# tangxyw/RecAlgorithm

Hardware: AMD Instinct MI355X
Metric: CTR examples/sec (train step fwd+bwd+TF1-Adam), batch 4096/GPU, 26 fields x emb16 (higher is better)
Workload: dtype f32; 1 GPU; DCN 3-layer CrossNet + MLP 512,256,128; 26 fields x emb16; batch 4096/GPU; data_batches=32, global_batch=4096, fields=26, emb_dim=16, embedding_rows=2790871, launch=hipGraph replay, parallelism=single

## Files before the change

recalgorithm_amd/_lib.py:

```python
from __future__ import annotations

import ctypes
import os
import re

from . import _abi
from ._abi import RecalgoError

_HERE = os.path.dirname(os.path.abspath(__file__))
LIB_PATH = os.environ.get("RECALGO_HIP_LIB") or os.path.join(_HERE, "librecalgo_hip.so")

P = ctypes.c_void_p


def _versioned(header: str):
    abi = _abi.read(header)
    defines = [c for c in abi.constants if re.fullmatch(r"RECALGO_(?:[A-Z0-9]+_)?ABI_VERSION", c)]
    queries = [f for f in abi.functions if re.fullmatch(r"recalgo_(?:[a-z0-9]+_)?abi_version", f)]
    if len(defines) != 1 or queries != [defines[0].lower()]:
        raise RecalgoError(f"include/{header}: a header of HEADERS has exactly one RECALGO_[<KEY>_]ABI_VERSION define and the "
                           f"one function recalgo_[<key>_]abi_version of the same key; found {defines} and {queries}")
    abi.version, abi.version_query = abi.constants[defines[0]], queries[0]
    abi.label = defines[0][len("RECALGO_"):-len("_VERSION")].replace("_", " ")
    return abi


HEADERS = {h: _versioned(h) for h in ("recalgo.h", "recalgo_cgc.h", "recalgo_wide.h", "recalgo_bst.h",
                                              "recalgo_res.h")}
MORE_HEADERS = {"recalgo_dien.h": _versioned("recalgo_dien.h")}
SERVING_HEADERS = {h: _versioned(h) for h in ("recalgo_serve.h", "recalgo_metrics.h", "recalgo_sumstep.h",
                                                      "recalgo_ragged.h", "recalgo_afm.h")}
ABI = HEADERS["recalgo.h"]
SIGNATURES = ABI.functions
STRUCTS = ABI.structs
CONSTANTS = ABI.constants
ABI_VERSION = ABI.version
_lib = None


def all_headers() -> dict:
    return {**HEADERS, **MORE_HEADERS}


def every_header() -> dict:
    return {**all_headers(), **SERVING_HEADERS}


def launch_errcheck(name: str):
    def errcheck(rc, func=None, args=None):
        check(rc, name)
        return rc
    return errcheck


# ... 30 lines not shown
```

recalgorithm_amd/csrc/sparse.hip:

```cpp
#include <cstddef>
#include <cstdlib>

#include "deferred.h"

#ifndef RECALGO_APPLY_WGS
#define RECALGO_APPLY_WGS 4
#endif
#ifndef RECALGO_APPLY_LDS_KEYS
#define RECALGO_APPLY_LDS_KEYS 2048
#endif
#ifndef RECALGO_APPLY_KU
#define RECALGO_APPLY_KU 8
#endif

namespace {

constexpr int kThreads = 256;
constexpr int kMaxSources = RECALGO_SCATTER_MAX_SOURCES;
using recalgo_deferred::kLrRing;
constexpr unsigned kLdsKeys = RECALGO_APPLY_LDS_KEYS;
constexpr unsigned kMaxSeg = kThreads;
constexpr unsigned kSlots = 512;
constexpr unsigned kLongSeg = 48;
constexpr unsigned kMaxLong = 64;
constexpr unsigned kCatchReq = 128;
constexpr unsigned long long kPadKey = ~0ull;
// ... 191 lines not shown

constexpr int kPrepSources = 4;
struct PrepareArgs {
    SrcDev S;
    SrcDev Sx[kPrepSources - 1];
    unsigned n_src;
    unsigned nreq_x[kPrepSources - 1];
    unsigned catch_end[kPrepSources];
    unsigned count_end[kPrepSources];
    unsigned* total;
    unsigned nb_log2, cs;
    Deferred D;
    Deferred D1;
    const long long* step;
    int step_off;
    unsigned K;
    unsigned n_req;
    unsigned b_catch, b_comp, b_count, b_sweep;
    long long rows, rows1;
    int period;
    unsigned passes, passes1;
    unsigned bshift, bshift1;
    int sweeping;
};

__device__ __forceinline__ long long request_row_linear(const SrcDev& S, unsigned r) {
    const unsigned e = r / S.F, f = r - e * S.F;
    return request_row(S, e, f);
}

__device__ __forceinline__ bool claim_row(int* last_step, long long row, int target, int* s_out) {
    const int s = __hip_atomic_load(&last_step[row], __ATOMIC_RELAXED, __HIP_MEMORY_SCOPE_AGENT);
    if (s > 0 && s < target && atomicCAS(&last_step[row], s, -s) == s) {
        *s_out = s;
        return true;
    }
    return false;
}

struct Claims {
    int* row; int* s;
    int* row2; int* s2;
    int* won;
    unsigned* hist;
    unsigned* n;
};
// ... 168 lines not shown
    int s = 0, old = 0;
    bool lag = false;
    long long row = -1;
    if (active && r < n_req) {
        row = request_row_linear(S, r);
        if (row >= 0 && row < n_rows && !(A.sweeping && (int)((row >> (8 + bshift)) % A.period) == cidx)) {
            s = __hip_atomic_load(&D.last_step[row], __ATOMIC_RELAXED, __HIP_MEMORY_SCOPE_AGENT);
            lag = s > 0 && s < target;
        }
    }
    if (lag) old = atomicCAS(&D.last_step[row], s, -s);
    unsigned slot = 0;
    if (lag) {
        slot = atomicAdd(C.n, 1u);
        C.row[slot] = (int)row;
        C.s[slot] = s;
    }
    __syncthreads();
    replay_claims(D, K, target, C, recalgo_deferred::lr_window(D.lr_ring, target), lag, slot, old, s);
}

__global__ __launch_bounds__(kThreads, 8) void sparse_prepare_kernel(PrepareArgs A) {
    extern __shared__ __attribute__((aligned(16))) unsigned lds_u[];
    const int target = A.D.last_step ? (int)(A.step[0] + A.step_off) : 0;
    const int cidx = A.period > 0 ? target % A.period : 0;
    if (blockIdx.x < A.b_catch) {
        if (A.n_src > 1) {
            unsigned si = 0, b0 = 0;
#pragma unroll
            for (int i = 1; i < kPrepSources; ++i)
                if ((unsigned)i < A.n_src && blockIdx.x >= A.catch_end[i - 1]) { si = i; b0 = A.catch_end[i - 1]; }
            SrcDev S = A.S;
            unsigned n_req = A.n_req;
#pragma unroll
            for (int i = 1; i < kPrepSources; ++i)
                if (si == (unsigned)i) { S = A.Sx[i - 1]; n_req = A.nreq_x[i - 1]; }
            catchup_requests(A, S, n_req, A.D, A.K, (blockIdx.x - b0) * kCatchReq + threadIdx.x, threadIdx.x < kCatchReq, A.rows, A.bshift,
                             cidx, target, claims_carve(lds_u));
            return;
        }
        catchup_requests(A, A.S, A.n_req, A.D, A.K, blockIdx.x * kCatchReq + threadIdx.x, threadIdx.x < kCatchReq, A.rows, A.bshift, cidx,
                         target, claims_carve(lds_u));
        return;
    }
    if (blockIdx.x < A.b_comp) {
        catchup_requests(A, A.S, A.n_req, A.D1, 1, (blockIdx.x - A.b_catch) * kThreads + threadIdx.x, true, A.rows1, A.bshift1, cidx,
// ... 14 lines not shown
            for (int i = 1; i < kPrepSources; ++i)
                if (si == (unsigned)i) S = A.Sx[i - 1];
            cb -= b0;
        }
        const unsigned li = cb * kThreads + threadIdx.x;
        unsigned e, f;
        const long long row = li < S.n ? slot_row(S, li, &e, &f) : -1;
        unsigned slot;
        const EqInfo eq = tile_equal(row >= 0 ? (unsigned)row : 0xffffffffu, hkey, mask, &slot);
        if (row >= 0 && eq.before == 0) atomicAdd(&A.total[(size_t)bucket_of((unsigned)row, A.nb_log2) << A.cs], 1u);
        return;
    }
    if (target <= 0) return;
    const Claims C = claims_carve(lds_u);
    if (blockIdx.x < A.b_sweep) {
        const recalgo_deferred::LrWindow W = recalgo_deferred::lr_window(A.D.lr_ring, target);
        const long long wg = blockIdx.x - A.b_count, nwg = A.b_sweep - A.b_count;
        sweep_units(A.D, A.K, A.passes, [&](unsigned pu) { return sweep_unit_row(cidx, A.period, A.bshift, wg + (long long)pu * nwg); },
                    A.rows, target, C, W);
        return;
    }
    {
        const recalgo_deferred::LrWindow W = recalgo_deferred::lr_window(A.D1.lr_ring, target);
        const long long wg = blockIdx.x - A.b_sweep, nwg = (long long)gridDim.x - A.b_sweep;
        sweep_units(A.D1, 1, A.passes1, [&](unsigned pu) { return sweep_unit_row(cidx, A.period, A.bshift1, wg + (long long)pu * nwg); },
                    A.rows1, target, C, W);
    }
}

struct PlaceArgs {
    SrcDev src[kMaxSources];
    int n_src;
    unsigned n_total;
    const unsigned* total; unsigned* cursor;
    unsigned cs;
    uint4* sched;
    const unsigned* offs_g; int prescanned;
    float* hdr;
    float* lr_ring; float* lr_ring1;
    const long long* step; int step_off;
    float lr, b1, b2;
    unsigned long long* keys;
    float* partials;
    float* partials1;
    unsigned nb_log2;
    unsigned KV, L;
    int stage_ok;
// ... 688 lines not shown

RECALGO_EXPORT int64_t recalgo_scatter_plan_header_bytes(int nb_log2) {
    if (!nb_ok(nb_log2)) return 0;
    return (32 + 2 * ((1ll << nb_log2) << counter_shift())) * (int64_t)sizeof(unsigned);
}

RECALGO_EXPORT int recalgo_scatter_plan_scan(void* plan_workspace, int64_t plan_requests, int nb_log2, recalgo_plan_scan_t* out) {
    RECALGO_REQUIRE(plan_workspace != nullptr && out != nullptr && nb_ok(nb_log2) && plan_requests >= 0 &&
                    plan_requests % kThreads == 0);
    const Ws ws = carve(plan_workspace, plan_requests, nb_log2);
    out->total = ws.total; out->offs = ws.offs; out->sched = ws.sched;
    out->counter_shift = counter_shift(); out->nb_log2 = (unsigned)nb_log2;
    return 0;
}

RECALGO_EXPORT int64_t recalgo_scatter_plan_workspace_bytes(int64_t n_slots, int nb_log2, int K) {
    if (n_slots < 0 || n_slots % kThreads != 0 || !nb_ok(nb_log2) || K < 1) return 0;
    const int64_t nb = 1ll << nb_log2;
    const int64_t cap = n_slots > 0 ? n_slots : kThreads;
    return (5 * nb + 2 * (nb << counter_shift()) + 32) * (int64_t)sizeof(unsigned) + 2 * cap * (int64_t)sizeof(unsigned long long) +
           cap * (int64_t)(K + 1) * (int64_t)sizeof(float) + 64;
}

static int scatter_prepare_impl(const recalgo_scatter_source_t* source, int n_sources, const int64_t* first_requests, int K,
                                void* plan_workspace, int64_t plan_requests, int nb_log2, int flags,
                                const recalgo_deferred_adam_t* deferred, const recalgo_deferred_adam_t* companion_deferred,
                                int64_t rows, int64_t companion_rows, int sweep_period, const int64_t* step_dev, int step_offset,
                                recalgo_stream_t stream);

RECALGO_EXPORT int recalgo_scatter_prepare(const recalgo_scatter_source_t* source, int K, void* plan_workspace,
                                           int64_t plan_requests, int nb_log2, int64_t first_request, int flags,
                                           const recalgo_deferred_adam_t* deferred,
                                           const recalgo_deferred_adam_t* companion_deferred, int64_t rows, int64_t companion_rows,
                                           int sweep_period, const int64_t* step_dev, int step_offset, recalgo_stream_t stream) {
    return scatter_prepare_impl(source, (source != nullptr && source->n_ex > 0) ? 1 : 0, &first_request, K, plan_workspace, plan_requests,
                                nb_log2, flags, deferred, companion_deferred, rows, companion_rows, sweep_period, step_dev, step_offset,
                                stream);
}

RECALGO_EXPORT int recalgo_scatter_prepare_multi(const recalgo_scatter_source_t* sources, int n_sources, const int64_t* first_requests,
                                                 int K, void* plan_workspace, int64_t plan_requests, int nb_log2, int flags,
                                                 const recalgo_deferred_adam_t* deferred, int64_t rows, int sweep_period,
                                                 const int64_t* step_dev, int step_offset, recalgo_stream_t stream) {
    RECALGO_REQUIRE(sources != nullptr && first_requests != nullptr && n_sources >= 1 && n_sources <= kPrepSources);
    for (int i = 0; i < n_sources; ++i) RECALGO_REQUIRE(sources[i].n_ex > 0);
    return scatter_prepare_impl(sources, n_sources, first_requests, K, plan_workspace, plan_requests, nb_log2, flags, deferred, nullptr,
                                rows, 0, sweep_period, step_dev, step_offset, stream);
}

static int scatter_prepare_impl(const recalgo_scatter_source_t* source, int n_sources, const int64_t* first_requests, int K,
                                void* plan_workspace, int64_t plan_requests, int nb_log2, int flags,
                                const recalgo_deferred_adam_t* deferred, const recalgo_deferred_adam_t* companion_deferred,
                                int64_t rows, int64_t companion_rows, int sweep_period, const int64_t* step_dev, int step_offset,
                                recalgo_stream_t stream) {
    RECALGO_REQUIRE(nb_ok(nb_log2) && plan_workspace != nullptr);
    RECALGO_REQUIRE(plan_requests >= 0 && plan_requests % kThreads == 0);
    RECALGO_REQUIRE(rows >= 0 && rows < (1ll << 31) && companion_rows >= 0 && companion_rows < (1ll << 31));
    const bool count = (flags & RECALGO_PREPARE_COUNT) != 0, sweep = (flags & RECALGO_PREPARE_SWEEP) != 0;
    const bool catchup = (flags & RECALGO_PREPARE_CATCHUP) != 0;
    const int64_t first_request = first_requests[0];
    RECALGO_REQUIRE(first_request >= 0 && first_request % kThreads == 0 && first_request < (1ll << 31));
    SrcDev S[kMaxSources];
    unsigned n = 0;
    if (n_sources >= 1) {
        RECALGO_REQUIRE(to_dev(source, 1, S, &n, false));
        RECALGO_REQUIRE(first_request + (int64_t)n <= plan_requests);
    } else {
        recalgo_scatter_source_t none{};
        to_dev(&none, 0, S, &n, false);
    }
    Geometry G;
    RECALGO_REQUIRE(geometry(K, nullptr, 0, &G));
    PrepareArgs A;
    A.S = S[0];
    A.S.first = (unsigned)first_request;
    A.n_src = n_sources > 1 ? (unsigned)n_sources : 1u;
    unsigned n_x[kPrepSources - 1] = {0, 0, 0};
// ... 33 lines not shown
    for (int i = 1; i < kPrepSources; ++i) {
        if (i < n_sources) {
            if (catchup) catch_blocks += (unsigned)cdiv(A.nreq_x[i - 1], kCatchReq);
            if (count) count_blocks += (unsigned)cdiv(n_x[i - 1], kThreads);
        }
        A.catch_end[i] = catch_blocks;
        A.count_end[i] = count_blocks;
    }
    A.period = sweep_period < 1 ? 1 : sweep_period;
    A.rows = rows; A.rows1 = companion_rows;
    A.bshift = sweep_block_shift(rows, A.period);
    A.bshift1 = sweep_block_shift(companion_rows, A.period);
    const long long brows = (long long)kThreads << A.bshift, brows1 = (long long)kThreads << A.bshift1;
    const long long share = cdiv(cdiv(rows, brows), A.period), share1 = cdiv(cdiv(companion_rows, brows1), A.period);
    A.passes = sweep_passes(share * brows);
    A.passes1 = sweep_passes(share1 * brows1);
    A.sweeping = sweep ? 1 : 0;
    const unsigned sweep_blocks = sweep ? (unsigned)cdiv(share * (brows / kSweepRows), (long long)A.passes) : 0u;
    const unsigned sweep1_blocks = (sweep && A.D1.last_step) ? (unsigned)cdiv(share1 * (brows1 / kSweepRows), (long long)A.passes1) : 0u;
    A.b_catch = catch_blocks;
    A.b_comp = A.b_catch + comp_blocks;
    A.b_count = A.b_comp + count_blocks;
    A.b_sweep = A.b_count + sweep_blocks;
    const unsigned blocks = A.b_sweep + sweep1_blocks;
    if (blocks == 0) return 0;
    const size_t smem = kSlots * 9 * sizeof(unsigned);
    static_assert(kClaimsLdsBytes <= kSlots * 9 * sizeof(unsigned), "claim lists fit the count tiles' LDS");
    hipLaunchKernelGGL(sparse_prepare_kernel, dim3(blocks), dim3(kThreads), smem, as_stream(stream), A);
    RECALGO_RETURN_LAST();
}

RECALGO_EXPORT int recalgo_scatter_apply(const recalgo_scatter_source_t* sources, int n_sources,
                                         const recalgo_scatter_companion_t* companion, int K, void* plan_workspace,
                                         int64_t plan_requests, int nb_log2, int mode, float* w, float* m, float* v,
                                         float* grad, const recalgo_deferred_adam_t* deferred, int64_t rows,
                                         const recalgo_live_t* live, const int64_t* step_dev,
                                         int step_offset, float lr, float beta1, float beta2, float eps,
                                         recalgo_stream_t stream) {
    RECALGO_REQUIRE(sources != nullptr && n_sources >= 1 && n_sources <= kMaxSources && plan_workspace != nullptr);
    RECALGO_REQUIRE(nb_ok(nb_log2) && rows >= 0 && rows < (1ll << 31));
    const int prescanned = (mode & RECALGO_SCATTER_PRESCANNED) != 0;
    mode &= ~RECALGO_SCATTER_PRESCANNED;
    RECALGO_REQUIRE(mode == RECALGO_SCATTER_GRAD || mode == RECALGO_SCATTER_ADAM || mode == RECALGO_SCATTER_LAZY_ADAM);
    RECALGO_REQUIRE(mode != RECALGO_SCATTER_GRAD ? (w && m && v && step_dev) : grad != nullptr);
    RECALGO_REQUIRE(mode != RECALGO_SCATTER_ADAM || (deferred && deferred->last_step && deferred->lr_ring));
    if (companion) {
        RECALGO_REQUIRE(companion->sources != nullptr && companion->rows >= 0 && companion->rows < (1ll << 31));
// ... 93 lines not shown
```

recalgorithm_amd/csrc/tail.hip:

```cpp
#include <algorithm>
#include <utility>
#include <vector>

#include "deferred.h"
#include "act.h"
#include "plan_scan.h"
#include "slab_sum.h"
#include "../../include/recalgo_sumstep.h"
#include "sigmoid_ce.h"

namespace {

__global__ __launch_bounds__(1024) void sigmoid_ce_kernel(
    const float* __restrict__ logits, const float* __restrict__ labels, unsigned B,
    float grad_scale, float* __restrict__ prob, float* __restrict__ loss,
    float* __restrict__ dlogit) {
    __shared__ float red[16];
    const float l = sigmoid_ce_task(
        logits, labels, B, grad_scale, dlogit != nullptr, red, [&](unsigned i, float p) { prob[i] = p; },
        [&](unsigned i, float d) { dlogit[i] = d; });
    if (threadIdx.x == 0) loss[0] = l;
}

using recalgo_deferred::adam1;

__global__ __launch_bounds__(256) void adam_tf1_kernel(float* __restrict__ p, float* __restrict__ g,
                                                       float* __restrict__ m, float* __restrict__ v,
                                                       int64_t n4, int64_t n, float lr_t_val,
                                                       const float* __restrict__ lr_t_dev, float b1,
                                                       float b2, float eps, int zero_grad) {
// ... 657 lines not shown
        A.x[p] = p < n_parts ? parts[p] : nullptr;
        A.width[p] = p < n_parts ? widths[p] : 0;
        A.off[p] = C;
        if (p < n_parts) {
            RECALGO_REQUIRE((parts[p] != nullptr || B == 0) && widths[p] >= 1);
            C += widths[p];
        }
    }
    A.n = n_parts; A.B = B; A.C = C; A.out = out; A.scale = scale; A.sum_out = sum_out;
    A.rows_per_block = 16;
    const int blocks = B > 0 ? cdiv(B, A.rows_per_block) : 1;
    A.ticket = static_cast<unsigned*>(workspace);
    A.partials = reinterpret_cast<float*>(static_cast<unsigned*>(workspace) + 16);
    hipLaunchKernelGGL(concat_sumsq_kernel, dim3(blocks), dim3(256), 0, as_stream(stream), A);
    RECALGO_RETURN_LAST();
}

namespace {
}

namespace {
__global__ __launch_bounds__(256) void copy_bytes_kernel(unsigned char* __restrict__ dst, const unsigned char* __restrict__ src,
                                                         size_t head, size_t n16, size_t nbytes) {
    const size_t t = (size_t)blockIdx.x * 256 + threadIdx.x, T = (size_t)gridDim.x * 256;
    const uint4* s16 = reinterpret_cast<const uint4*>(src + head);
    uint4* d16 = reinterpret_cast<uint4*>(dst + head);
    size_t i = t;
    for (; i + 3 * T < n16; i += 4 * T) {
        const uint4 a = s16[i], b = s16[i + T], c = s16[i + 2 * T], d = s16[i + 3 * T];
        d16[i] = a; d16[i + T] = b; d16[i + 2 * T] = c; d16[i + 3 * T] = d;
    }
    for (; i < n16; i += T) d16[i] = s16[i];
    if (t < head) dst[t] = src[t];
    const size_t tail0 = head + n16 * 16;
    if (tail0 + t < nbytes && t < 16) dst[tail0 + t] = src[tail0 + t];
}
}

RECALGO_EXPORT int recalgo_copy_bytes(void* dst, const void* src, int64_t nbytes, recalgo_stream_t stream) {
    RECALGO_REQUIRE(nbytes >= 0 && (nbytes == 0 || (dst != nullptr && src != nullptr)));
    if (nbytes == 0) return 0;
    const uintptr_t d = reinterpret_cast<uintptr_t>(dst), s = reinterpret_cast<uintptr_t>(src);
    size_t head = 0, n16 = 0;
    if ((d & 15) == (s & 15)) {
        head = (16 - (d & 15)) & 15;
        if (head > (size_t)nbytes) head = (size_t)nbytes;
        n16 = ((size_t)nbytes - head) / 16;
    } else {
        return (int)hipMemcpyAsync(dst, src, (size_t)nbytes, hipMemcpyDeviceToDevice, as_stream(stream));
    }
    const size_t want = (n16 + 255) / 256;
    const unsigned blocks = (unsigned)(want < 1 ? 1 : (want > 2048 ? 2048 : want));
    hipLaunchKernelGGL(copy_bytes_kernel, dim3(blocks), dim3(256), 0, as_stream(stream), static_cast<unsigned char*>(dst),
                       static_cast<const unsigned char*>(src), head, n16, (size_t)nbytes);
    RECALGO_RETURN_LAST();
}

RECALGO_EXPORT int recalgo_abi_version(void) { return RECALGO_ABI_VERSION; }
RECALGO_EXPORT const char* recalgo_target_arch(void) { return "gfx950"; }

RECALGO_EXPORT int recalgo_sigmoid_ce_fwd_bwd(const float* logits, const float* labels, int B,
                                              float grad_scale, float* prob, float* loss,
                                              float* dlogit, recalgo_stream_t stream) {
    RECALGO_REQUIRE(B > 0);
    hipLaunchKernelGGL(sigmoid_ce_kernel, dim3(1), dim3(1024), 0, as_stream(stream), logits, labels,
                       (unsigned)B, grad_scale, prob, loss, dlogit);
    RECALGO_RETURN_LAST();
}

RECALGO_EXPORT int recalgo_adam_tf1_advance(int64_t* step_dev, float lr, float beta1, float beta2,
                                            float* lr_t_dev, recalgo_stream_t stream) {
    RECALGO_REQUIRE(step_dev != nullptr && lr_t_dev != nullptr);
    hipLaunchKernelGGL(adam_advance_kernel, dim3(1), dim3(64), 0, as_stream(stream), step_dev, lr, beta1,
                       beta2, lr_t_dev);
    RECALGO_RETURN_LAST();
// ... 328 lines not shown
```

recalgorithm_amd/estimator.py:

```python
from __future__ import annotations

import os
import time
from typing import Callable, Dict, Iterable, Optional

import torch

from . import ops
from .variables import VariableStore, use_store


class ModeKeys:
    TRAIN = "train"
    EVAL = "eval"
    PREDICT = "infer"


class EstimatorSpec:
    def __init__(self, mode, predictions=None, loss=None, train_op=None, eval_metric_ops=None,
                 export_outputs=None, training_hooks=None, **_ignored):
        self.mode, self.predictions, self.loss, self.train_op = mode, predictions, loss, train_op
        self.eval_metric_ops = eval_metric_ops
        self.export_outputs, self.training_hooks = export_outputs, training_hooks


RAGGED_AUTO_MARGIN = (5, 4)
RAGGED_AUTO_ROUND = 1024


def check_ragged_capacity(policy):
    ok = policy is None or policy == "auto" or (isinstance(policy, int) and not isinstance(policy, bool) and policy >= 1) or \
# ... 440 lines not shown
        st = t.untyped_storage()
        key = st.data_ptr()
        lo, hi = spans[key]
        lo -= lo % 16
        if key not in storages:
            part = torch.empty(0, dtype=torch.uint8, device=t.device).set_(st, lo, (max(hi - lo, 0),), (1,))
            storages[key] = part.clone().untyped_storage()
        off = t.storage_offset() - lo // t.element_size()
        return torch.empty(0, dtype=t.dtype, device=t.device).set_(storages[key], off, t.shape, t.stride())

    def walk(o):
        if isinstance(o, torch.Tensor):
            return cl(o)
        if isinstance(o, Ragged):
            return Ragged(cl(o.values), cl(o.offsets))
        if isinstance(o, dict):
            return {k: walk(v) for k, v in o.items()}
        if isinstance(o, (tuple, list)):
            return type(o)(walk(v) for v in o)
        return o
    return walk(obj)


HOUSEKEEPING_EVERY = 32
OVERFLOW_POLL_EVERY = 64


def _quiesce_collectives() -> None:
    try:
        import torch.distributed as dist
        if not (dist.is_available() and dist.is_initialized()) or dist.get_backend() != "nccl":
            return
    except Exception:
        return
    import time
    torch.cuda.synchronize()
    time.sleep(0.5)


class BatchShapeMismatch(ValueError):
    """A batch whose structure / shapes are not those the step was captured on (the last partial batch of an epoch): the
    ONLY condition under which the training loop runs a step eagerly beside a captured graph — any other error of the
    replay path propagates."""


class GraphedTrainStep:

    pad_values = False

    def __init__(self, step_fn: Callable, features, labels, warmup: int = 3):
        self.step_fn = step_fn
        span = getattr(features, "device_span", None)
        features, labels = _clone_tree((features, labels))
        self.static_f, self.static_l = features, labels
        self._static = list(_tree_tensors(features, "f")) + list(_tree_tensors(labels, "l"))
        self._span_plan = None
        if span is not None and self._static:
            st0 = self._static[0][1].untyped_storage()
            if (st0.nbytes() >= span[0].numel() and all(t.untyped_storage().data_ptr() == st0.data_ptr() for _, t in self._static)
                    and all(a.storage_offset() == b.storage_offset() and a.stride() == b.stride() and a.shape == b.shape
                            for (_, a), (_, b) in zip(self._static, list(_tree_tensors(span[2][0], "f")) + list(_tree_tensors(span[2][1], "l"))))):
                dst = torch.empty(0, dtype=torch.uint8, device=span[0].device).set_(st0, 0, (span[0].numel(),), (1,))
                self._span_plan = (span[1], dst)
        s = torch.cuda.Stream()
        s.wait_stream(torch.cuda.current_stream())
        with torch.cuda.stream(s):
            for _ in range(warmup):
                self.out = step_fn(features, labels)
        torch.cuda.current_stream().wait_stream(s)
        torch.cuda.synchronize()
        _quiesce_collectives()
        self.graph = torch.cuda.CUDAGraph()
        with torch.cuda.graph(self.graph, capture_error_mode="thread_local"):
            self.out = step_fn(features, labels)
        self.warmup_steps = warmup
        owner = getattr(step_fn, "__self__", None)
        self._housekeeping = getattr(getattr(owner, "store", None), "housekeeping", None)
        self._calls = 0

    def load(self, features, labels):
        span = getattr(features, "device_span", None)
        if span is not None and self._span_plan is not None and span[1] == self._span_plan[0]:
            _device_copy(self._span_plan[1], span[0])
            return
        new = list(_tree_tensors(features, "f")) + list(_tree_tensors(labels, "l"))
        if len(new) != len(self._static):
            raise BatchShapeMismatch("graphed step: the input structure changed")
        spans = self._static_spans()
        groups = {}
        pads = []
        for i, ((k0, dst), (k1, src)) in enumerate(zip(self._static, new)):
            if k0 != k1 or dst.shape != src.shape:
                if (self.pad_values and k0 == k1 and k1.endswith(".values") and src.dim() == 1 and src.numel() <= dst.numel()
                        and src.dtype == dst.dtype == torch.int64 and src.device == dst.device and src.is_cuda):
                    pads.append((dst, src))
                    continue
                raise BatchShapeMismatch(f"graphed step: input {k1} changed shape/structure")
            if dst.dtype == src.dtype and dst.stride() == src.stride() and src.device == dst.device:
                groups.setdefault((spans[i][0], src.untyped_storage().data_ptr()), []).append((i, src.storage_offset() * spans[i][3]))
            else:
                dst.copy_(src, non_blocking=True)
        singles = []
        for items in groups.values():
            if len(items) > 1:
                d_lo = min(spans[i][1] for i, _ in items)
                d_hi = max(spans[i][2] for i, _ in items)
                s_lo = min(lo for _, lo in items)
                mine = {i for i, _ in items}
                st_ptr = spans[items[0][0]][0]
                alone = all(k in mine or sp[0] != st_ptr or sp[2] <= d_lo or sp[1] >= d_hi for k, sp in enumerate(spans))
                if alone and d_hi > d_lo and all(spans[i][1] - d_lo == lo - s_lo for i, lo in items):
                    d0, s0 = self._static[items[0][0]][1], new[items[0][0]][1]
                    dv = self._dst_views.get((spans[items[0][0]][0], d_lo, d_hi))
                    if dv is None:
                        dv = torch.empty(0, dtype=torch.uint8, device=d0.device).set_(d0.untyped_storage(), d_lo, (d_hi - d_lo,), (1,))
                        self._dst_views[(spans[items[0][0]][0], d_lo, d_hi)] = dv
                    sv = torch.empty(0, dtype=torch.uint8, device=s0.device).set_(s0.untyped_storage(), s_lo, (d_hi - d_lo,), (1,))
                    _device_copy(dv, sv)
                    continue
            singles.extend(i for i, _ in items)
        for i in singles:
            self._static[i][1].copy_(new[i][1], non_blocking=True)
        for dst, src in pads:
            ops.ragged_pad(src.contiguous(), dst.numel(), out=dst)

    def _static_spans(self):
        sp = self.__dict__.get("_spans")
        if sp is None:
            sp = self._spans = [(t.untyped_storage().data_ptr(),) + _byte_span(t) + (t.element_size(),) for _, t in self._static]
            self._dst_views = {}
        return sp

    def __call__(self, features=None, labels=None):
        if features is not None:
            self.load(features, labels)
        self.graph.replay()
        self._calls += 1
        if self._housekeeping is not None and self._calls % HOUSEKEEPING_EVERY == 0:
            self._housekeeping()
        return self.out


def _device_copy(dst: torch.Tensor, src: torch.Tensor) -> None:
    if dst.is_cuda and src.is_cuda and dst.device == src.device and dst.is_contiguous() and src.is_contiguous():
        from . import ops
        ops.copy_bytes(dst, src)
    else:
        dst.copy_(src, non_blocking=True)


def _host_copy(dst: torch.Tensor, src: torch.Tensor) -> None:
    if (dst.dtype == src.dtype and dst.numel() == src.numel() and dst.is_contiguous() and src.is_contiguous()
            and dst.device.type == "cpu" and src.device.type == "cpu"):
        import ctypes
        ctypes.memmove(dst.data_ptr(), src.data_ptr(), dst.numel() * dst.element_size())
    else:
        dst.copy_(src)

# ... 153 lines not shown
        if len(keys) < 2 or set(features) != set(keys) or mat.dtype != torch.int64 or not mat.is_contiguous() or mat.device.type != "cpu":
            return None
        B = mat.shape[0]
        labs = list(labels.items())
        if not all(isinstance(v, torch.Tensor) and v.device.type == "cpu" and v.dtype == torch.float32 and v.numel() == B
                   for _, v in labs):
            return None
        nid = mat.numel() * 8
        total = nid + 4 * B * len(labs)
        sig = ("ids+labels", int(total), int(B), tuple(keys), tuple(k for k, _ in labs), tuple(tuple(v.shape) for _, v in labs))

        def fill(buf):
            _host_copy(buf[:nid].view(torch.int64).view(mat.shape), mat)
            for i, (_, v) in enumerate(labs):
                _host_copy(buf[nid + 4 * B * i:nid + 4 * B * (i + 1)].view(torch.float32), v.reshape(-1))
        return mat, keys, labs, nid, total, sig, fill

    def feed_step(self, graphed: "GraphedTrainStep", features, labels, pb=None):
        plan = graphed._span_plan
        if plan is not None:
            pb = pb if pb is not None else self._packed_host_batch(features, labels)
            if pb is not None and pb[5] == plan[0] and plan[1].numel() == pb[4]:
                self._h2d(pb[6], (pb[4],), torch.uint8, dst=plan[1])
                return graphed()
        features, labels = self._to_device(features, labels)
        return graphed(features, labels)

    def _pack_host_columns(self, features: dict, force: bool = False) -> dict:
        if self.device.type == "cpu" and not force:
            return features
        groups = {"ids": [], "dense": []}
        for k in sorted(features):
            v = features[k]
            if not isinstance(v, torch.Tensor) or v.device.type != "cpu":
                continue
            if v.dtype == torch.int64 and v.dim() == 1:
                groups["ids"].append(k)
            elif v.dtype == torch.float32 and v.dim() == 2 and v.shape[1] == 1:
                groups["dense"].append(k)
        out = dict(features)
        packed = getattr(features, "packed_ids", None)
        if packed is not None and len(packed[1]) >= 2 and packed[1] == groups["ids"] and all(
                features[k].data_ptr() == packed[0][:, j].data_ptr() and features[k].stride() == packed[0][:, j].stride()
                for j, k in enumerate(packed[1])):
            mat = packed[0]
            dev = self._h2d(lambda buf: _host_copy(buf, mat), tuple(mat.shape), torch.int64) if self.device.type == "cuda" \
# ... 496 lines not shown
```

recalgorithm_amd/sparse.py:

```python
from __future__ import annotations

import ctypes
import os
from typing import List, Optional

import torch

from . import _lib

_C = _lib.CONSTANTS
MODE_GRAD, MODE_ADAM, MODE_LAZY_ADAM = _C["RECALGO_SCATTER_GRAD"], _C["RECALGO_SCATTER_ADAM"], _C["RECALGO_SCATTER_LAZY_ADAM"]
MODE_PRESCANNED = _C["RECALGO_SCATTER_PRESCANNED"]
PREPARE_COUNT, PREPARE_SWEEP, PREPARE_CATCHUP = _C["RECALGO_PREPARE_COUNT"], _C["RECALGO_PREPARE_SWEEP"], _C["RECALGO_PREPARE_CATCHUP"]
MAX_SOURCES = _C["RECALGO_SCATTER_MAX_SOURCES"]
LR_RING = _C["RECALGO_LR_RING"]
_CSource, _CCompanion = _lib.STRUCTS["recalgo_scatter_source_t"], _lib.STRUCTS["recalgo_scatter_companion_t"]
_CPlanScan, _CDeferred = _lib.STRUCTS["recalgo_plan_scan_t"], _lib.STRUCTS["recalgo_deferred_adam_t"]
_CLookupJob = _lib.STRUCTS["recalgo_lookup_job_t"]


SCATTER_MODE = "owner"
COMPANION = True
NB_LOG2 = None

# ... 141 lines not shown
    K = arena.K
    return arena.weight.shape[0] < (1 << 31) and ((K % 4 == 0 and K // 4 <= 64) or K <= 64)


def plan_of(arena) -> Optional[ArenaPlan]:
    return getattr(arena, "sparse", None)


def view_for(src, arena, store):
    if src is not None and src.caught_up:
        return None, None
    return deferred_view(arena, store)


def deferred_view(arena, store):
    plan = plan_of(arena)
    if plan is None or plan.last_step is None or store is None or getattr(store, "opt_state", None) is None:
        return None, None
    d = plan._deferred_struct()
    plan._view = d
    return ctypes.byref(d), ctypes.c_void_p(store.opt_state["step"].data_ptr())


def begin_lookup(arena, store, ids: torch.Tensor, offsets: Optional[torch.Tensor], row_base: Optional[torch.Tensor],
                 base: int, n_ex: int, F: int, training: Optional[bool] = None, companion_arena=None,
                 can_defer: bool = False) -> Optional[Source]:
    plan = plan_of(arena)
    if training is None:
        training = torch.is_grad_enabled()
    training = bool(training) and getattr(arena, "trainable", True)
    if not (training and scatter_mode() == "owner" and _supported(arena)):
        return None
    if plan is None:
        plan = arena.sparse = ArenaPlan(arena)
    if plan.companions:
        _dissolve(plan)
    src = Source(ids, offsets, row_base, base, n_ex, F)
    src.arena = arena
    if src.n == 0:
        plan.sources.append(src)
        return src
    lib = _lib.load()
    first = sum(s.slots for s in plan.sources)
    if plan.ws is None or first + src.slots > plan.capacity:
        plan._ensure_ws(first + src.slots)
    if plan.counted is None or plan.counted[:2] != (plan.ws.data_ptr(), plan.nb_log2):
        plan.clear_counts()
    cs = src.c_struct(arena.K)
    d = plan._deferred_struct()
    src.caught_up = True
    step = None if d is None else store.opt_state["step"]
    d1, c_rows = None, 0
    if companion_arena is not None and _pair(src, arena, companion_arena) and d is not None:
        cp = plan_of(companion_arena)
        d1 = cp._deferred_struct()
        c_rows = companion_arena.weight.shape[0] if d1 is not None else 0
    flags = (0 if d is None else PREPARE_CATCHUP) | PREPARE_COUNT
    if d is not None and not plan.swept:
        flags |= PREPARE_SWEEP
        plan.swept = True
        if d1 is not None:
            plan_of(companion_arena).swept = True
    if (_batch is not None and can_defer and d1 is None and companion_arena is None and getattr(arena, "sharding", None) is None
            and "__staged__" not in getattr(arena, "tables", {})):
        src.deferred = True
        _batch["arenas"].setdefault(id(arena), (arena, plan, []))[2].append((src, cs, first, flags, d, step))
    elif flags:
        lib.recalgo_scatter_prepare(ctypes.byref(cs), arena.K, ctypes.c_void_p(plan.ws.data_ptr()), plan.capacity, plan.nb_log2,
                                    first, flags, None if d is None else ctypes.byref(d),
                                    None if d1 is None else ctypes.byref(d1), arena.weight.shape[0], c_rows, sweep_period(),
                                    None if step is None else ctypes.c_void_p(step.data_ptr()), 0, _stream(arena.weight))
    plan.sources.append(src)
    plan.counted = plan.counted[:2] + (plan.counted[2] + (id(src),),)
    return src


_batch = None
MAX_PREPARE_SOURCES = 4
BATCH_LOOKUPS = True


class batch_lookups:

    def __enter__(self):
        global _batch
        self.prev = _batch
        if BATCH_LOOKUPS:
            _batch = {"arenas": {}, "launches": []}
        return self
# ... 15 lines not shown
def defer_launch(fn, job=None) -> None:
    _batch["launches"].append((fn, job))


def flush_batch() -> None:
    global _batch
    if _batch is not None and (_batch["arenas"] or _batch["launches"]):
        b, _batch = _batch, {"arenas": {}, "launches": []}
        _flush_batch(b)


def _flush_batch(b) -> None:
    lib = _lib.load()
    for arena, plan, entries in b["arenas"].values():
        for i in range(0, len(entries), MAX_PREPARE_SOURCES):
            chunk = entries[i:i + MAX_PREPARE_SOURCES]
            flags = 0
            for e in chunk:
                flags |= e[3]
            d = next((e[4] for e in chunk if e[4] is not None), None)
            step = next((e[5] for e in chunk if e[5] is not None), None)
            ws = ctypes.c_void_p(plan.ws.data_ptr())
            stp = None if step is None else ctypes.c_void_p(step.data_ptr())
            if len(chunk) == 1:
                _, cs, first, _, _, _ = chunk[0]
                lib.recalgo_scatter_prepare(ctypes.byref(cs), arena.K, ws, plan.capacity, plan.nb_log2, first, flags,
                                            None if d is None else ctypes.byref(d), None, arena.weight.shape[0], 0,
                                            sweep_period(), stp, 0, _stream(arena.weight))
            else:
                arr = (_CSource * len(chunk))(*[e[1] for e in chunk])
                firsts = (ctypes.c_int64 * len(chunk))(*[e[2] for e in chunk])
                lib.recalgo_scatter_prepare_multi(arr, len(chunk), firsts, arena.K, ws, plan.capacity, plan.nb_log2, flags,
                                                  None if d is None else ctypes.byref(d), arena.weight.shape[0],
                                                  sweep_period(), stp, 0, _stream(arena.weight))
                prepare_stats["merged"] += len(chunk) - 1
        have = set(plan.counted[2]) | {id(e[0]) for e in entries}
        plan.counted = plan.counted[:2] + (tuple(id(s) for s in plan.sources if id(s) in have),)
    plain = [(fn, job) for fn, job in b["launches"] if job is not None]
    for fn, job in b["launches"]:
        if job is None:
            fn()
    for i in range(0, len(plain), 4):
        chunk = plain[i:i + 4]
        if len(chunk) == 1:
            chunk[0][0]()
            continue
        ptr = lambda t: None if t is None else t.data_ptr()
        arr = (_CLookupJob * len(chunk))(*[_CLookupJob(j[0], ptr(j[1]), ptr(j[2]), ptr(j[3]), j[4], j[5], j[6], ptr(j[7]), j[8], j[9],
# ... 94 lines not shown
        grads.append(g.reshape(-1, K))
    allrows = torch.cat(rows).reshape(-1, 1).contiguous()
    merged = Source(allrows, None, None, 0, allrows.shape[0], 1)
    merged.set_grad(torch.cat(grads).contiguous())
    return rest + [merged]


def plan_scan_record(arena, lazy: bool):
    plan = plan_of(arena)
    if plan is None or plan.ws is None or plan.companions or (plan.served and not plan.sources):
        return None
    srcs = [s for s in plan.sources if s.g is not None and s.n]
    if not srcs or len(srcs) > MAX_SOURCES or sum(s.slots for s in srcs) > plan.capacity or plan.counted != plan._signature(srcs):
        return None
    rec = _CPlanScan()
    _lib.check(_lib.load().recalgo_scatter_plan_scan(ctypes.c_void_p(plan.ws.data_ptr()), plan.capacity, plan.nb_log2,
                                                     ctypes.byref(rec)), "recalgo_scatter_plan_scan")
    plan.prescanned = plan._signature(srcs)
    return rec


def _run(plan: ArenaPlan, sources: List[Source], mode: int, step_dev, step_offset: int, lr: float, live=None):
    lib = _lib.load()
    prescanned, plan.prescanned = plan.prescanned, None
    a = plan.arena
    comp_arena = _companion_arena(sources, mode)
    if len([s for s in sources if s.n]) > MAX_SOURCES:
        if comp_arena is not None:
            _dissolve(plan_of(comp_arena))
            comp_arena = None
        sources = _merge_dense(sources, a.K)
    srcs = [s for s in sources if s.n]
    plan._ensure_ws(sum(s.slots for s in srcs))
    if not srcs or prescanned != plan._signature(srcs) or plan.counted != prescanned:
        prescanned = None
    if plan.counted != plan._signature(srcs):
        if plan.counted is None or plan.counted[2] or plan.counted[:2] != (plan.ws.data_ptr(), plan.nb_log2):
            plan.clear_counts()
        first = 0
        for s in srcs:
            cs = s.c_struct(a.K)
            lib.recalgo_scatter_prepare(ctypes.byref(cs), a.K, ctypes.c_void_p(plan.ws.data_ptr()), plan.capacity,
                                        plan.nb_log2, first, PREPARE_COUNT, None, None, 0, 0, 1, None, 0, _stream(a.weight))
            first += s.slots
    if not srcs:
        dummy = Source(a.weight, None, None, 0, 0, 1)
# ... 172 lines not shown
```

Measured before the change: 20.68 million examples/s.

## Fuse input feed copy into sparse prepare kernel launched ahead of graph replay

Moves the first sparse-prepare launch out of the captured hipGraph into a separate 'head' launch issued before each replay. That head kernel also carries extra blocks that perform the device-to-device copy of the batch id span into the static input buffer. The prepare blocks read the ids straight from the source buffer via pointer offsets, so the standalone copy kernel and its dependency ahead of prepare go away. The cost is one extra host launch per step outside the graph, plus more complex bookkeeping that patches source pointers and must stay correct.

```diff
diff --git a/include/recalgo_feed.h b/include/recalgo_feed.h
--- /dev/null
+++ b/include/recalgo_feed.h
@@ -0,0 +1,26 @@
+#ifndef RECALGO_FEED_H_
+#define RECALGO_FEED_H_
+
+#include <stdint.h>
+
+#ifdef __cplusplus
+extern "C" {
+#endif
+
+typedef void* recalgo_stream_t;
+
+#define RECALGO_FEED_ABI_VERSION 1
+int recalgo_feed_abi_version(void);
+
+int recalgo_scatter_prepare_feed_supported(const void* feed_dst, const void* feed_src, int64_t feed_bytes);
+int recalgo_scatter_prepare_feed(const void* sources, int n_sources, const int64_t* first_requests, int K, void* plan_workspace,
+                                 int64_t plan_requests, int nb_log2, int flags, const void* deferred,
+                                 const void* companion_deferred, int64_t rows, int64_t companion_rows, int sweep_period,
+                                 const int64_t* step_dev, int step_offset, void* feed_dst, const void* feed_src,
+                                 int64_t feed_bytes, recalgo_stream_t stream);
+
+#ifdef __cplusplus
+}
+#endif
+
+#endif
diff --git a/recalgorithm_amd/_lib.py b/recalgorithm_amd/_lib.py
--- a/recalgorithm_amd/_lib.py
+++ b/recalgorithm_amd/_lib.py
@@ -29,7 +29,7 @@
                                               "recalgo_res.h")}
 MORE_HEADERS = {"recalgo_dien.h": _versioned("recalgo_dien.h")}
 SERVING_HEADERS = {h: _versioned(h) for h in ("recalgo_serve.h", "recalgo_metrics.h", "recalgo_sumstep.h",
-                                                      "recalgo_ragged.h", "recalgo_afm.h")}
+                                                      "recalgo_ragged.h", "recalgo_afm.h", "recalgo_feed.h")}
 ABI = HEADERS["recalgo.h"]
 SIGNATURES = ABI.functions
 STRUCTS = ABI.structs
diff --git a/recalgorithm_amd/csrc/copy_span.h b/recalgorithm_amd/csrc/copy_span.h
--- /dev/null
+++ b/recalgorithm_amd/csrc/copy_span.h
@@ -0,0 +1,40 @@
+#pragma once
+
+#include <cstddef>
+#include <cstdint>
+
+#include <hip/hip_runtime.h>
+
+namespace recalgo_copy {
+
+__device__ __forceinline__ void copy_span(unsigned char* __restrict__ dst, const unsigned char* __restrict__ src, size_t head, size_t n16,
+                                          size_t nbytes, size_t t, size_t T) {
+    const uint4* s16 = reinterpret_cast<const uint4*>(src + head);
+    uint4* d16 = reinterpret_cast<uint4*>(dst + head);
+    size_t i = t;
+    for (; i + 3 * T < n16; i += 4 * T) {
+        const uint4 a = s16[i], b = s16[i + T], c = s16[i + 2 * T], d = s16[i + 3 * T];
+        d16[i] = a; d16[i + T] = b; d16[i + 2 * T] = c; d16[i + 3 * T] = d;
+    }
+    for (; i < n16; i += T) d16[i] = s16[i];
+    if (t < head) dst[t] = src[t];
+    const size_t tail0 = head + n16 * 16;
+    if (tail0 + t < nbytes && t < 16) dst[tail0 + t] = src[tail0 + t];
+}
+
+inline bool copy_span_split(const void* dst, const void* src, size_t nbytes, size_t* head, size_t* n16) {
+    const uintptr_t d = reinterpret_cast<uintptr_t>(dst), s = reinterpret_cast<uintptr_t>(src);
+    if ((d & 15) != (s & 15)) return false;
+    size_t h = (16 - (d & 15)) & 15;
+    if (h > nbytes) h = nbytes;
+    *head = h;
+    *n16 = (nbytes - h) / 16;
+    return true;
+}
+
+inline unsigned copy_span_blocks(size_t n16) {
+    const size_t want = (n16 + 255) / 256;
+    return (unsigned)(want < 1 ? 1 : (want > 2048 ? 2048 : want));
+}
+
+}
diff --git a/recalgorithm_amd/csrc/sparse.hip b/recalgorithm_amd/csrc/sparse.hip
--- a/recalgorithm_amd/csrc/sparse.hip
+++ b/recalgorithm_amd/csrc/sparse.hip
@@ -2,6 +2,8 @@
 #include <cstdlib>
 
 #include "deferred.h"
+#include "copy_span.h"
+#include "../../include/recalgo_feed.h"
 
 #ifndef RECALGO_APPLY_WGS
 #define RECALGO_APPLY_WGS 4
@@ -239,6 +241,9 @@
     unsigned passes, passes1;
     unsigned bshift, bshift1;
     int sweeping;
+    unsigned b_copy;
+    unsigned char* feed_dst; const unsigned char* feed_src;
+    size_t feed_head, feed_n16, feed_bytes;
 };
 
 __device__ __forceinline__ long long request_row_linear(const SrcDev& S, unsigned r) {
@@ -453,6 +458,11 @@
 
 __global__ __launch_bounds__(kThreads, 8) void sparse_prepare_kernel(PrepareArgs A) {
     extern __shared__ __attribute__((aligned(16))) unsigned lds_u[];
+    if (blockIdx.x >= A.b_copy) {
+        recalgo_copy::copy_span(A.feed_dst, A.feed_src, A.feed_head, A.feed_n16, A.feed_bytes,
+                                (size_t)(blockIdx.x - A.b_copy) * kThreads + threadIdx.x, (size_t)(gridDim.x - A.b_copy) * kThreads);
+        return;
+    }
     const int target = A.D.last_step ? (int)(A.step[0] + A.step_off) : 0;
     const int cidx = A.period > 0 ? target % A.period : 0;
     if (blockIdx.x < A.b_catch) {
@@ -513,7 +523,7 @@
     }
     {
         const recalgo_deferred::LrWindow W = recalgo_deferred::lr_window(A.D1.lr_ring, target);
-        const long long wg = blockIdx.x - A.b_sweep, nwg = (long long)gridDim.x - A.b_sweep;
+        const long long wg = blockIdx.x - A.b_sweep, nwg = (long long)A.b_copy - A.b_sweep;
         sweep_units(A.D1, 1, A.passes1, [&](unsigned pu) { return sweep_unit_row(cidx, A.period, A.bshift1, wg + (long long)pu * nwg); },
                     A.rows1, target, C, W);
     }
@@ -1248,11 +1258,13 @@
            cap * (int64_t)(K + 1) * (int64_t)sizeof(float) + 64;
 }
 
+struct Feed { void* dst = nullptr; const void* src = nullptr; size_t bytes = 0; };
+
 static int scatter_prepare_impl(const recalgo_scatter_source_t* source, int n_sources, const int64_t* first_requests, int K,
                                 void* plan_workspace, int64_t plan_requests, int nb_log2, int flags,
                                 const recalgo_deferred_adam_t* deferred, const recalgo_deferred_adam_t* companion_deferred,
                                 int64_t rows, int64_t companion_rows, int sweep_period, const int64_t* step_dev, int step_offset,
-                                recalgo_stream_t stream);
+                                recalgo_stream_t stream, const Feed& feed);
 
 RECALGO_EXPORT int recalgo_scatter_prepare(const recalgo_scatter_source_t* source, int K, void* plan_workspace,
                                            int64_t plan_requests, int nb_log2, int64_t first_request, int flags,
@@ -1261,7 +1273,7 @@
                                            int sweep_period, const int64_t* step_dev, int step_offset, recalgo_stream_t stream) {
     return scatter_prepare_impl(source, (source != nullptr && source->n_ex > 0) ? 1 : 0, &first_request, K, plan_workspace, plan_requests,
                                 nb_log2, flags, deferred, companion_deferred, rows, companion_rows, sweep_period, step_dev, step_offset,
-                                stream);
+                                stream, Feed{});
 }
 
 RECALGO_EXPORT int recalgo_scatter_prepare_multi(const recalgo_scatter_source_t* sources, int n_sources, const int64_t* first_requests,
@@ -1271,14 +1283,53 @@
     RECALGO_REQUIRE(sources != nullptr && first_requests != nullptr && n_sources >= 1 && n_sources <= kPrepSources);
     for (int i = 0; i < n_sources; ++i) RECALGO_REQUIRE(sources[i].n_ex > 0);
     return scatter_prepare_impl(sources, n_sources, first_requests, K, plan_workspace, plan_requests, nb_log2, flags, deferred, nullptr,
-                                rows, 0, sweep_period, step_dev, step_offset, stream);
+                                rows, 0, sweep_period, step_dev, step_offset, stream, Feed{});
+}
+
+static int feed_check(const void* dst, const void* src, int64_t nbytes) {
+    if (nbytes < 0) return -1;
+    if (src == nullptr || nbytes == 0 || dst == src) return 0;
+    if (dst == nullptr) return -1;
+    const uintptr_t d = reinterpret_cast<uintptr_t>(dst), s = reinterpret_cast<uintptr_t>(src), n = (uintptr_t)nbytes;
+    if ((d & 15) != (s & 15)) return -1;
+    if (d < s ? s - d < n : d - s < n) return -1;
+    return 1;
+}
+
+RECALGO_EXPORT int recalgo_feed_abi_version(void) { return RECALGO_FEED_ABI_VERSION; }
+
+RECALGO_EXPORT int recalgo_scatter_prepare_feed_supported(const void* feed_dst, const void* feed_src, int64_t feed_bytes) {
+    return feed_check(feed_dst, feed_src, feed_bytes) >= 0 ? 1 : 0;
+}
+
+RECALGO_EXPORT int recalgo_scatter_prepare_feed(const void* sources, int n_sources, const int64_t* first_requests, int K,
+                                                void* plan_workspace, int64_t plan_requests, int nb_log2, int flags,
+                                                const void* deferred, const void* companion_deferred, int64_t rows,
+                                                int64_t companion_rows, int sweep_period, const int64_t* step_dev, int step_offset,
+                                                void* feed_dst, const void* feed_src, int64_t feed_bytes, recalgo_stream_t stream) {
+    const recalgo_scatter_source_t* src = static_cast<const recalgo_scatter_source_t*>(sources);
+    const recalgo_deferred_adam_t* d = static_cast<const recalgo_deferred_adam_t*>(deferred);
+    const recalgo_deferred_adam_t* d1 = static_cast<const recalgo_deferred_adam_t*>(companion_deferred);
+    const int fc = feed_check(feed_dst, feed_src, feed_bytes);
+    RECALGO_REQUIRE(fc >= 0 && n_sources >= 0 && n_sources <= kPrepSources && (n_sources == 0 || (src != nullptr && first_requests != nullptr)));
+    Feed feed;
+    if (fc > 0) { feed.dst = feed_dst; feed.src = feed_src; feed.bytes = (size_t)feed_bytes; }
+    const int64_t zero = 0;
+    if (n_sources <= 1)
+        return scatter_prepare_impl(src, (n_sources == 1 && src->n_ex > 0) ? 1 : 0, n_sources == 1 ? first_requests : &zero, K,
+                                    plan_workspace, plan_requests, nb_log2, flags, d, d1, rows, companion_rows, sweep_period, step_dev,
+                                    step_offset, stream, feed);
+    RECALGO_REQUIRE(d1 == nullptr && companion_rows == 0);
+    for (int i = 0; i < n_sources; ++i) RECALGO_REQUIRE(src[i].n_ex > 0);
+    return scatter_prepare_impl(src, n_sources, first_requests, K, plan_workspace, plan_requests, nb_log2, flags, d, nullptr, rows, 0,
+                                sweep_period, step_dev, step_offset, stream, feed);
 }
 
 static int scatter_prepare_impl(const recalgo_scatter_source_t* source, int n_sources, const int64_t* first_requests, int K,
                                 void* plan_workspace, int64_t plan_requests, int nb_log2, int flags,
                                 const recalgo_deferred_adam_t* deferred, const recalgo_deferred_adam_t* companion_deferred,
                                 int64_t rows, int64_t companion_rows, int sweep_period, const int64_t* step_dev, int step_offset,
-                                recalgo_stream_t stream) {
+                                recalgo_stream_t stream, const Feed& feed) {
     RECALGO_REQUIRE(nb_ok(nb_log2) && plan_workspace != nullptr);
     RECALGO_REQUIRE(plan_requests >= 0 && plan_requests % kThreads == 0);
     RECALGO_REQUIRE(rows >= 0 && rows < (1ll << 31) && companion_rows >= 0 && companion_rows < (1ll << 31));
@@ -1358,7 +1409,17 @@
     A.b_comp = A.b_catch + comp_blocks;
     A.b_count = A.b_comp + count_blocks;
     A.b_sweep = A.b_count + sweep_blocks;
-    const unsigned blocks = A.b_sweep + sweep1_blocks;
+    A.b_copy = A.b_sweep + sweep1_blocks;
+    A.feed_dst = static_cast<unsigned char*>(feed.dst);
+    A.feed_src = static_cast<const unsigned char*>(feed.src);
+    A.feed_head = A.feed_n16 = 0;
+    A.feed_bytes = feed.dst != nullptr ? feed.bytes : 0;
+    unsigned copy_blocks = 0;
+    if (A.feed_bytes > 0) {
+        RECALGO_REQUIRE(recalgo_copy::copy_span_split(feed.dst, feed.src, A.feed_bytes, &A.feed_head, &A.feed_n16));
+        copy_blocks = recalgo_copy::copy_span_blocks(A.feed_n16);
+    }
+    const unsigned blocks = A.b_copy + copy_blocks;
     if (blocks == 0) return 0;
     const size_t smem = kSlots * 9 * sizeof(unsigned);
     static_assert(kClaimsLdsBytes <= kSlots * 9 * sizeof(unsigned), "claim lists fit the count tiles' LDS");
diff --git a/recalgorithm_amd/csrc/tail.hip b/recalgorithm_amd/csrc/tail.hip
--- a/recalgorithm_amd/csrc/tail.hip
+++ b/recalgorithm_amd/csrc/tail.hip
@@ -6,6 +6,7 @@
 #include "act.h"
 #include "plan_scan.h"
 #include "slab_sum.h"
+#include "copy_span.h"
 #include "../../include/recalgo_sumstep.h"
 #include "sigmoid_ce.h"
 
@@ -709,35 +710,18 @@
 namespace {
 __global__ __launch_bounds__(256) void copy_bytes_kernel(unsigned char* __restrict__ dst, const unsigned char* __restrict__ src,
                                                          size_t head, size_t n16, size_t nbytes) {
-    const size_t t = (size_t)blockIdx.x * 256 + threadIdx.x, T = (size_t)gridDim.x * 256;
-    const uint4* s16 = reinterpret_cast<const uint4*>(src + head);
-    uint4* d16 = reinterpret_cast<uint4*>(dst + head);
-    size_t i = t;
-    for (; i + 3 * T < n16; i += 4 * T) {
-        const uint4 a = s16[i], b = s16[i + T], c = s16[i + 2 * T], d = s16[i + 3 * T];
-        d16[i] = a; d16[i + T] = b; d16[i + 2 * T] = c; d16[i + 3 * T] = d;
-    }
-    for (; i < n16; i += T) d16[i] = s16[i];
-    if (t < head) dst[t] = src[t];
-    const size_t tail0 = head + n16 * 16;
-    if (tail0 + t < nbytes && t < 16) dst[tail0 + t] = src[tail0 + t];
+    recalgo_copy::copy_span(dst, src, head, n16, nbytes, (size_t)blockIdx.x * 256 + threadIdx.x, (size_t)gridDim.x * 256);
 }
 }
 
 RECALGO_EXPORT int recalgo_copy_bytes(void* dst, const void* src, int64_t nbytes, recalgo_stream_t stream) {
     RECALGO_REQUIRE(nbytes >= 0 && (nbytes == 0 || (dst != nullptr && src != nullptr)));
     if (nbytes == 0) return 0;
-    const uintptr_t d = reinterpret_cast<uintptr_t>(dst), s = reinterpret_cast<uintptr_t>(src);
     size_t head = 0, n16 = 0;
-    if ((d & 15) == (s & 15)) {
-        head = (16 - (d & 15)) & 15;
-        if (head > (size_t)nbytes) head = (size_t)nbytes;
-        n16 = ((size_t)nbytes - head) / 16;
-    } else {
+    if (!recalgo_copy::copy_span_split(dst, src, (size_t)nbytes, &head, &n16)) {
         return (int)hipMemcpyAsync(dst, src, (size_t)nbytes, hipMemcpyDeviceToDevice, as_stream(stream));
     }
-    const size_t want = (n16 + 255) / 256;
-    const unsigned blocks = (unsigned)(want < 1 ? 1 : (want > 2048 ? 2048 : want));
+    const unsigned blocks = recalgo_copy::copy_span_blocks(n16);
     hipLaunchKernelGGL(copy_bytes_kernel, dim3(blocks), dim3(256), 0, as_stream(stream), static_cast<unsigned char*>(dst),
                        static_cast<const unsigned char*>(src), head, n16, (size_t)nbytes);
     RECALGO_RETURN_LAST();
diff --git a/recalgorithm_amd/estimator.py b/recalgorithm_amd/estimator.py
--- a/recalgorithm_amd/estimator.py
+++ b/recalgorithm_amd/estimator.py
@@ -6,7 +6,7 @@
 
 import torch
 
-from . import ops
+from . import _lib, ops
 from .variables import VariableStore, use_store
 
 
@@ -493,6 +493,7 @@
     return walk(obj)
 
 
+FEED_IN_PREPARE = True
 HOUSEKEEPING_EVERY = 32
 OVERFLOW_POLL_EVERY = 64
 
@@ -518,6 +519,8 @@
 class GraphedTrainStep:
 
     pad_values = False
+    _head = _feed = None
+    head_launches = fused_feeds = 0
 
     def __init__(self, step_fn: Callable, features, labels, warmup: int = 3):
         self.step_fn = step_fn
@@ -542,8 +545,20 @@
         torch.cuda.synchronize()
         _quiesce_collectives()
         self.graph = torch.cuda.CUDAGraph()
-        with torch.cuda.graph(self.graph, capture_error_mode="thread_local"):
-            self.out = step_fn(features, labels)
+        from . import sparse
+        rec = None
+        if FEED_IN_PREPARE:
+            storages = {t.untyped_storage().data_ptr(): t.untyped_storage().nbytes() for _, t in self._static if t.is_cuda}
+            rec = sparse.HeadRecorder(storages.items())
+        prev, sparse.head_recorder = sparse.head_recorder, rec
+        try:
+            with torch.cuda.graph(self.graph, capture_error_mode="thread_local"):
+                self.out = step_fn(features, labels)
+        finally:
+            sparse.head_recorder = prev
+        if rec is not None:
+            self._head = rec.head
+        self._feed_ok = {}
         self.warmup_steps = warmup
         owner = getattr(step_fn, "__self__", None)
         self._housekeeping = getattr(getattr(owner, "store", None), "housekeeping", None)
@@ -551,8 +566,11 @@
 
     def load(self, features, labels):
         span = getattr(features, "device_span", None)
+        self._feed = None
         if span is not None and self._span_plan is not None and span[1] == self._span_plan[0]:
-            _device_copy(self._span_plan[1], span[0])
+            dst = self._span_plan[1]
+            if not self._feed_through_head(dst.data_ptr(), span[0], span[0].data_ptr(), dst.numel()):
+                _device_copy(dst, span[0])
             return
         new = list(_tree_tensors(features, "f")) + list(_tree_tensors(labels, "l"))
         if len(new) != len(self._static):
@@ -587,7 +605,8 @@
                         dv = torch.empty(0, dtype=torch.uint8, device=d0.device).set_(d0.untyped_storage(), d_lo, (d_hi - d_lo,), (1,))
                         self._dst_views[(spans[items[0][0]][0], d_lo, d_hi)] = dv
                     sv = torch.empty(0, dtype=torch.uint8, device=s0.device).set_(s0.untyped_storage(), s_lo, (d_hi - d_lo,), (1,))
-                    _device_copy(dv, sv)
+                    if not self._feed_through_head(dv.data_ptr(), sv, sv.data_ptr(), d_hi - d_lo):
+                        _device_copy(dv, sv)
                     continue
             singles.extend(i for i, _ in items)
         for i in singles:
@@ -595,6 +614,21 @@
         for dst, src in pads:
             ops.ragged_pad(src.contiguous(), dst.numel(), out=dst)
 
+    def _feed_through_head(self, dst: int, keep: torch.Tensor, src: int, nbytes: int) -> bool:
+        h = self._head
+        if h is None or self._feed is not None or not (dst <= h.span_ptr + h.lo and h.span_ptr + h.hi <= dst + nbytes):
+            return False
+        ok = self._feed_ok.get((dst, src, nbytes))
+        if ok is None:
+            if len(self._feed_ok) >= 256:
+                self._feed_ok.clear()
+            ok = self._feed_ok[(dst, src, nbytes)] = (
+                dst != src and keep.is_cuda and keep.device == h.arena.weight.device and keep.is_contiguous()
+                and bool(_lib.load().recalgo_scatter_prepare_feed_supported(dst, src, nbytes)))
+        if ok:
+            self._feed = (dst, src, nbytes, keep)
+        return ok
+
     def _static_spans(self):
         sp = self.__dict__.get("_spans")
         if sp is None:
@@ -605,6 +639,11 @@
     def __call__(self, features=None, labels=None):
         if features is not None:
             self.load(features, labels)
+        if self._head is not None:
+            feed, self._feed = self._feed, None
+            self._head.launch(feed)
+            self.head_launches += 1
+            self.fused_feeds += feed is not None
         self.graph.replay()
         self._calls += 1
         if self._housekeeping is not None and self._calls % HOUSEKEEPING_EVERY == 0:
@@ -804,6 +843,7 @@
             pb = pb if pb is not None else self._packed_host_batch(features, labels)
             if pb is not None and pb[5] == plan[0] and plan[1].numel() == pb[4]:
                 self._h2d(pb[6], (pb[4],), torch.uint8, dst=plan[1])
+                graphed._feed = None
                 return graphed()
         features, labels = self._to_device(features, labels)
         return graphed(features, labels)
diff --git a/recalgorithm_amd/sparse.py b/recalgorithm_amd/sparse.py
--- a/recalgorithm_amd/sparse.py
+++ b/recalgorithm_amd/sparse.py
@@ -187,6 +187,77 @@
     return ctypes.byref(d), ctypes.c_void_p(store.opt_state["step"].data_ptr())
 
 
+head_recorder = None
+
+
+class StepHead:
+
+    def __init__(self, arena, entries, flags, d, d1, c_rows, step, span_ptr):
+        self.arena, self.span_ptr = arena, span_ptr
+        plan = plan_of(arena)
+        self.n = len(entries)
+        self._keep = (entries, d, d1, step, plan.ws)
+        self.arr = (_CSource * self.n)(*[cs for _, cs, _ in entries])
+        self.firsts = (ctypes.c_int64 * self.n)(*[first for _, _, first in entries])
+        self.static_ids = [src.ids.data_ptr() for src, _, _ in entries]
+        self.offs = [p - span_ptr for p in self.static_ids]
+        self.lo = min(self.offs)
+        self.hi = max(o + src.ids.numel() * 8 for o, (src, _, _) in zip(self.offs, entries))
+        self.dst, self.src = ctypes.c_void_p(None), ctypes.c_void_p(None)
+        self.fn = _lib.load().recalgo_scatter_prepare_feed
+        self.args = [self.arr, self.n, self.firsts, arena.K, ctypes.c_void_p(plan.ws.data_ptr()), plan.capacity, plan.nb_log2, flags,
+                     None if d is None else ctypes.byref(d), None if d1 is None else ctypes.byref(d1), arena.weight.shape[0], c_rows,
+                     sweep_period(), None if step is None else ctypes.c_void_p(step.data_ptr()), 0, self.dst, self.src, 0, None]
+        self.fed = False
+
+    def launch(self, feed=None) -> None:
+        a = self.args
+        if feed is not None:
+            dst, src, n = feed[:3]
+            delta = src - dst
+            for i in range(self.n):
+                self.arr[i].ids = self.static_ids[i] + delta
+            self.dst.value, self.src.value, a[17] = dst, src, n
+            self.fed = True
+        elif self.fed:
+            for i in range(self.n):
+                self.arr[i].ids = self.static_ids[i]
+            self.src.value, a[17] = None, 0
+            self.fed = False
+        a[18] = _stream(self.arena.weight)
+        self.fn(*a)
+
+
+class HeadRecorder:
+
+    def __init__(self, spans):
+        self.spans = [(int(p), int(n)) for p, n in spans]
+        self.head: Optional[StepHead] = None
+        self.closed = False
+
+    def close(self) -> None:
+        self.closed = True
+
+    def take(self, arena, entries, flags, d, d1, c_rows, step, clean: bool = True) -> bool:
+        if self.closed:
+            return False
+        self.closed = True
+        if not (clean and flags and 1 <= len(entries) <= MAX_PREPARE_SOURCES and (len(entries) == 1 or d1 is None)):
+            return False
+        if getattr(arena, "sharding", None) is not None or "__staged__" in getattr(arena, "tables", {}):
+            return False
+        at = entries[0][0].ids.data_ptr() if isinstance(entries[0][0].ids, torch.Tensor) else -1
+        lo, nbytes = next(((p, n) for p, n in self.spans if p <= at < p + n), (0, 0))
+        hi = lo + nbytes
+        for src, _, _ in entries:
+            ids = src.ids
+            if (src.offsets is not None or ids is None or src.n == 0 or ids.dtype != torch.int64 or not ids.is_contiguous()
+                    or not (lo <= ids.data_ptr() and ids.data_ptr() + ids.numel() * 8 <= hi)):
+                return False
+        self.head = StepHead(arena, entries, flags, d, d1, c_rows, step, lo)
+        return True
+
+
 def begin_lookup(arena, store, ids: torch.Tensor, offsets: Optional[torch.Tensor], row_base: Optional[torch.Tensor],
                  base: int, n_ex: int, F: int, training: Optional[bool] = None, companion_arena=None,
                  can_defer: bool = False) -> Optional[Source]:
@@ -207,10 +278,13 @@
         return src
     lib = _lib.load()
     first = sum(s.slots for s in plan.sources)
+    clean = True
     if plan.ws is None or first + src.slots > plan.capacity:
         plan._ensure_ws(first + src.slots)
+        clean = False
     if plan.counted is None or plan.counted[:2] != (plan.ws.data_ptr(), plan.nb_log2):
         plan.clear_counts()
+        clean = False
     cs = src.c_struct(arena.K)
     d = plan._deferred_struct()
     src.caught_up = True
@@ -229,7 +303,9 @@
     if (_batch is not None and can_defer and d1 is None and companion_arena is None and getattr(arena, "sharding", None) is None
             and "__staged__" not in getattr(arena, "tables", {})):
         src.deferred = True
-        _batch["arenas"].setdefault(id(arena), (arena, plan, []))[2].append((src, cs, first, flags, d, step))
+        _batch["arenas"].setdefault(id(arena), (arena, plan, []))[2].append((src, cs, first, flags, d, step, clean))
+    elif flags and head_recorder is not None and head_recorder.take(arena, [(src, cs, first)], flags, d, d1, c_rows, step, clean):
+        pass
     elif flags:
         lib.recalgo_scatter_prepare(ctypes.byref(cs), arena.K, ctypes.c_void_p(plan.ws.data_ptr()), plan.capacity, plan.nb_log2,
                                     first, flags, None if d is None else ctypes.byref(d),
@@ -291,8 +367,11 @@
             step = next((e[5] for e in chunk if e[5] is not None), None)
             ws = ctypes.c_void_p(plan.ws.data_ptr())
             stp = None if step is None else ctypes.c_void_p(step.data_ptr())
-            if len(chunk) == 1:
-                _, cs, first, _, _, _ = chunk[0]
+            if head_recorder is not None and head_recorder.take(arena, [e[:3] for e in chunk], flags, d, None, 0, step,
+                                                                all(e[6] for e in chunk)):
+                prepare_stats["merged"] += len(chunk) - 1
+            elif len(chunk) == 1:
+                _, cs, first = chunk[0][:3]
                 lib.recalgo_scatter_prepare(ctypes.byref(cs), arena.K, ws, plan.capacity, plan.nb_log2, first, flags,
                                             None if d is None else ctypes.byref(d), None, arena.weight.shape[0], 0,
                                             sweep_period(), stp, 0, _stream(arena.weight))
@@ -433,6 +512,8 @@
 
 def _run(plan: ArenaPlan, sources: List[Source], mode: int, step_dev, step_offset: int, lr: float, live=None):
     lib = _lib.load()
+    if head_recorder is not None:
+        head_recorder.close()
     prescanned, plan.prescanned = plan.prescanned, None
     a = plan.arena
     comp_arena = _companion_arena(sources, mode)
```

Measured after the change: 21.10 million examples/s (median of 6 runs). +2.0%, better.
